# ecker-lab/TreeLearn

Measured on AMD Instinct MI355X. Metric: Mpoints/sec through sparse U-Net fwd (0.1 m voxel, 40x40 m tile), higher is better.
Workload: dtype bf16; 1 GPU; config2: single 40x40 m tile, voxel 0.1 m, 1890607 points/tile, 7-level 32-ch sparse U-Net fwd (30.1 M params, random init), 1 tile per GPU; points_per_tile=1890607, tiles_in_flight=4

## Files before the change

### treelearn_amd/csrc/tl_blk.hip

```cpp
#include "tl_common.h"

namespace {

constexpr int kBlock = 256;
constexpr int HASH = 2048;
constexpr uint32_t EMPTY = 0xFFFFFFFFu;
constexpr uint32_t KEYMASK = 0x01FFFFFFu;
constexpr int LIST = 128;

struct BlkGrid { int B, BX, BY, BZ, TX, TY; int64_t nblk; };

__device__ __forceinline__ void blk_decode(const BlkGrid& g, int64_t blk, int& b, int& bx, int& by, int& bz) {
  bz = (int)(blk % g.BZ); blk /= g.BZ;
  const int iy = (int)(blk & 3), ix = (int)((blk >> 2) & 3); blk >>= 4;
  const int ty = (int)(blk % g.TY); blk /= g.TY;
  const int tx = (int)(blk % g.TX);
  b = (int)(blk / g.TX);
  bx = tx * 4 + ix; by = ty * 4 + iy;
}

__device__ __forceinline__ uint32_t wg_exclusive_scan(uint32_t v, uint32_t* total) {
  __shared__ uint32_t wsum[kBlock / 64];
  const int lane = threadIdx.x & 63, wid = threadIdx.x >> 6;
  uint32_t inc = v;
  for (int off = 1; off < 64; off <<= 1) {
    const uint32_t t = (uint32_t)__shfl_up((int)inc, off);
    if (lane >= off) inc += t;
  }
  if (lane == 63) wsum[wid] = inc;
  __syncthreads();
  uint32_t base = 0, tot = 0;
  for (int w = 0; w < kBlock / 64; ++w) { if (w < wid) base += wsum[w]; tot += wsum[w]; }
  __syncthreads();
  *total = tot;
  return base + inc - v;
}

__global__ void __launch_bounds__(kBlock) k_blk_count(const uint64_t* __restrict__ bm, TlDims d, BlkGrid g, uint32_t* __restrict__ cnt,
                                                      uint32_t* __restrict__ part) {
  const int64_t blk = (int64_t)blockIdx.x * kBlock + threadIdx.x;
  uint32_t c = 0;
  if (blk < g.nblk) {
    int b, bx, by, bz;
    blk_decode(g, blk, b, bx, by, bz);
    const int sh = (bz & 7) * 8;
    for (int xi = 0; xi < 8; ++xi) {
      const int x = bx * 8 + xi;
      if (x >= d.X) break;
      for (int yi = 0; yi < 8; ++yi) {
        const int y = by * 8 + yi;
        if (y >= d.Y) break;
        const uint64_t w = bm[tl_col_word(d, b, x, y) + (bz >> 3)];
        c += __popc((uint32_t)(w >> sh) & 0xFFu);
      }
    }
    cnt[blk] = c;
  }
  uint32_t tot;
  wg_exclusive_scan(c, &tot);
  if (threadIdx.x == 0) part[blockIdx.x] = tot;
}

__global__ void __launch_bounds__(kBlock) k_blk_starts(const uint32_t* __restrict__ cnt, const uint32_t* __restrict__ part_excl, int64_t nblk,
                                                       uint32_t* __restrict__ bstart) {
  const int64_t blk = (int64_t)blockIdx.x * kBlock + threadIdx.x;
  const uint32_t c = blk < nblk ? cnt[blk] : 0;
  uint32_t tot;
  const uint32_t ex = wg_exclusive_scan(c, &tot);
  if (blk < nblk) bstart[blk] = part_excl[blockIdx.x] + ex;
}

__global__ void __launch_bounds__(1024) k_scan_u32(const uint32_t* __restrict__ in, int64_t n, uint32_t* __restrict__ out, uint32_t* __restrict__ total) {
  __shared__ uint32_t wsum[16];
  const int tid = threadIdx.x, lane = tid & 63, wid = tid >> 6;
  const int64_t per = (n + 1023) / 1024, lo = (int64_t)tid * per, hi = lo + per < n ? lo + per : n;
  uint32_t s = 0;
  for (int64_t i = lo; i < hi; ++i) s += in[i];
  uint32_t inc = s;
  for (int off = 1; off < 64; off <<= 1) {
    const uint32_t t = (uint32_t)__shfl_up((int)inc, off);
    if (lane >= off) inc += t;
  }
  if (lane == 63) wsum[wid] = inc;
  __syncthreads();
  uint32_t base = 0, tot = 0;
  for (int w = 0; w < 16; ++w) { if (w < wid) base += wsum[w]; tot += wsum[w]; }
  uint32_t run = base + inc - s;
  for (int64_t i = lo; i < hi; ++i) { const uint32_t v = in[i]; out[i] = run; run += v; }
  if (tid == 0 && total) *total = tot;
}

__global__ void __launch_bounds__(kBlock) k_blk_order(const uint64_t* __restrict__ bm, const uint32_t* __restrict__ pf, TlDims d, BlkGrid g,
                                                      const uint32_t* __restrict__ cnt, const uint32_t* __restrict__ bstart,
                                                      int32_t* __restrict__ o2n, int32_t* __restrict__ perm, int32_t* __restrict__ coords_new,
                                                      uint32_t* __restrict__ cs) {
  const int lane = threadIdx.x & 63;
  const int64_t blk = (int64_t)blockIdx.x * (kBlock / 64) + (threadIdx.x >> 6);
  if (blk >= g.nblk) return;
  if (cnt[blk] == 0) return;
  int b, bx, by, bz;
  blk_decode(g, blk, b, bx, by, bz);
  const int x = bx * 8 + (lane >> 3), y = by * 8 + (lane & 7);
  const bool valid = x < d.X && y < d.Y;
  const int sh = (bz & 7) * 8;
  uint64_t word = 0; int64_t w = 0;
  if (valid) { w = tl_col_word(d, b, x, y) + (bz >> 3); word = bm[w]; }
  uint32_t byte = (uint32_t)(word >> sh) & 0xFFu;
  const uint32_t pc = __popc(byte);
  uint32_t inc = pc;
  for (int off = 1; off < 64; off <<= 1) {
    const uint32_t t = (uint32_t)__shfl_up((int)inc, off);
    if (lane >= off) inc += t;
  }
  if (!pc) return;
  int newr = (int)(bstart[blk] + inc - pc);
  int old = (int)(pf[w] + __popcll(word & ((1ull << sh) - 1ull)));
  cs[(((int64_t)b * d.X + x) * d.Y + y) * g.BZ + bz] = (uint32_t)newr;
  while (byte) {
    const int zb = __ffs((int)byte) - 1;
    byte &= byte - 1;
    o2n[old] = newr; perm[newr] = old;
    reinterpret_cast<int4*>(coords_new)[newr] = make_int4(b, x, y, bz * 8 + zb);
    ++old; ++newr;
  }
}

struct BlkOut {
  const uint32_t* cs; int BZ;
  const int32_t* coords_new;
  int32_t* unit; int32_t* counter;
  int32_t* halo; uint32_t* lrb; int32_t* pmask; int32_t* nn_out;
  int64_t n; int64_t nchunks; int64_t cap_units; int halo_max;
};

__global__ void __launch_bounds__(kBlock) k_blk_units(const uint64_t* __restrict__ bm, TlDims d, BlkOut p) {
  __shared__ uint32_t s_tab[kBlock / 64][HASH + 64];
  __shared__ uint32_t s_list[kBlock / 64][LIST];
  __shared__ uint32_t s_lslot[kBlock / 64][LIST];
  const int lane = threadIdx.x & 63, wv = threadIdx.x >> 6;
  const int64_t chunk = (int64_t)blockIdx.x * (kBlock / 64) + wv;
  if (chunk >= p.nchunks) return;
  uint32_t* tab = s_tab[wv];
  uint32_t* list = s_list[wv];
  uint32_t* lslot = s_lslot[wv];
  const int64_t base = chunk * 64;
  const int cnt = (int)(p.n - base < 64 ? p.n - base : 64);
  const int64_t r = base + lane;
  const bool rvalid = lane < cnt;

  int nn[27];
#pragma unroll
  for (int k = 0; k < 27; ++k) nn[k] = -1;
  uint32_t pm = 0;
  {
    const int4 c = rvalid ? reinterpret_cast<const int4*>(p.coords_new)[r] : make_int4(0, 0, 0, 0);
    const int z = c.w;
    const bool hz0 = z > 0, hz2 = z + 1 < d.Z;
    const int bA = (hz0 ? z - 1 : z) >> 3, bB = (hz2 ? z + 1 : z) >> 3;
    const bool x0 = hz0 && ((z - 1) >> 6) != (z >> 6), x2 = hz2 && ((z + 1) >> 6) != (z >> 6);
    const int64_t wc0 = rvalid ? tl_col_word(d, c.x, c.y, c.z) : 0;
    const int64_t ci0 = rvalid ? (((int64_t)c.x * d.X + c.y) * d.Y + c.z) * p.BZ : 0;
    const bool xin[3] = {rvalid && c.y > 0, rvalid, rvalid && c.y + 1 < d.X}, yin[3] = {c.z > 0, true, c.z + 1 < d.Y};
    const int zw1 = rvalid ? (z >> 6) : 0, zw0 = (rvalid && x0) ? ((z - 1) >> 6) : zw1, zw2 = (rvalid && x2) ? ((z + 1) >> 6) : zw1;
    bool inb[9];
    uint64_t w1[9];
#pragma unroll
    for (int q = 0; q < 9; ++q) {
      const int dx = q / 3 - 1, dy = q % 3 - 1;
      inb[q] = xin[q / 3] && yin[q % 3];
      w1[q] = bm[wc0 + (inb[q] ? (dx * d.Y + dy) * d.Zw : 0) + zw1];
    }
    uint32_t by3[9];
#pragma unroll
    for (int q = 0; q < 9; ++q) {
      const uint32_t b1 = (uint32_t)(w1[q] >> (z & 56)) & 0xFFu;
      const uint32_t b0 = (uint32_t)(w1[q] >> ((hz0 ? z - 1 : z) & 56)) & 0xFFu, b2 = (uint32_t)(w1[q] >> ((hz2 ? z + 1 : z) & 56)) & 0xFFu;
      by3[q] = b0 | (b1 << 8) | (b2 << 16);
    }
    if (__any(x0 || x2)) {
#pragma unroll
      for (int q = 0; q < 9; ++q) {
        const int dx = q / 3 - 1, dy = q % 3 - 1;
        const int64_t wcq = wc0 + (inb[q] ? (dx * d.Y + dy) * d.Zw : 0);
        const uint64_t a0 = bm[wcq + zw0], a2 = bm[wcq + zw2];
        if (x0) by3[q] = (by3[q] & ~0xFFu) | ((uint32_t)(a0 >> ((z - 1) & 56)) & 0xFFu);
        if (x2) by3[q] = (by3[q] & ~0xFF0000u) | (((uint32_t)(a2 >> ((z + 1) & 56)) & 0xFFu) << 16);
      }
    }
    bool p0[9], p1[9], p2[9];
    uint32_t sA[9], sB[9];
#pragma unroll
    for (int q = 0; q < 9; ++q) {
      const int dx = q / 3 - 1, dy = q % 3 - 1;
      p0[q] = inb[q] && hz0 && ((by3[q] >> ((z - 1) & 7)) & 1u);
      p1[q] = inb[q] && ((by3[q] >> (8 + (z & 7))) & 1u);
      p2[q] = inb[q] && hz2 && ((by3[q] >> (16 + ((z + 1) & 7))) & 1u);
      const bool any = p0[q] || p1[q] || p2[q];
      const int64_t ciq = ci0 + (inb[q] ? (dx * d.Y + dy) * p.BZ : 0);
      sA[q] = p.cs[any ? ciq + bA : 0];
      sB[q] = p.cs[(any && bB != bA) ? ciq + bB : 0];
    }
    auto rowid = [](uint32_t byte, int zz, uint32_t start) __attribute__((always_inline)) {
      return (int)(start + __popc(byte & ((1u << (zz & 7)) - 1u)));
    };
#pragma unroll
    for (int q = 0; q < 9; ++q) {
      const uint32_t b_ = bB != bA ? sB[q] : sA[q];
      if (p0[q]) { nn[3 * q] = rowid(by3[q] & 0xFFu, z - 1, sA[q]); pm |= 1u << (3 * q); }
      if (p1[q]) { nn[3 * q + 1] = rowid((by3[q] >> 8) & 0xFFu, z, (z >> 3) == bA ? sA[q] : b_); pm |= 2u << (3 * q); }
      if (p2[q]) { nn[3 * q + 2] = rowid((by3[q] >> 16) & 0xFFu, z + 1, b_); pm |= 4u << (3 * q); }
    }
    if (rvalid) {
      p.pmask[r] = (int32_t)pm;
      if (p.nn_out) {
#pragma unroll
        for (int k = 0; k < 27; ++k) p.nn_out[(int64_t)k * p.n + r] = nn[k];
      }
    }
  }

  int nref = __popc(pm);
  for (int off = 32; off > 0; off >>= 1) nref += __shfl_xor(nref, off);
  const int TS = nref <= 360 ? 512 : (nref <= 720 ? 1024 : HASH);
  const int tshift = nref <= 360 ? 23 : (nref <= 720 ? 22 : 21);
  auto hs = [&](int v) __attribute__((always_inline)) { return ((uint32_t)v * 2654435761u) >> tshift; };

  int st_a[8], st_e[8];
  int sp = 1;
  st_a[0] = 0; st_e[0] = cnt;
  bool first = true;
  while (sp > 0) {
    --sp;
    const int a = st_a[sp], e = st_e[sp];
    const int lo = (int)base + a, hi = (int)base + e;
    for (int i = lane; i < TS; i += 64) tab[i] = EMPTY;
    __builtin_amdgcn_fence(__ATOMIC_ACQ_REL, "workgroup");
    const bool inr = lane >= a && lane < e;
    uint32_t outm = 0;
#pragma unroll
    for (int k = 0; k < 27; ++k) {
      const int v = nn[k];
      const bool out = inr && v >= 0 && (v < lo || v >= hi);
      outm |= out ? (1u << k) : 0u;
      tab[out ? hs(v) : (uint32_t)TS] = (uint32_t)v;
    }
    __builtin_amdgcn_fence(__ATOMIC_ACQ_REL, "workgroup");
    uint32_t lost = 0;
#pragma unroll
    for (int k = 0; k < 27; ++k) {
      const uint32_t cur = tab[hs(nn[k])];
      lost |= (((outm >> k) & 1u) && cur != (uint32_t)nn[k]) ? (1u << k) : 0u;
    }
    if (__any(lost != 0)) {
#pragma unroll
      for (int k = 0; k < 27; ++k) {
        bool todo = (lost >> k) & 1u;
        if (__any(todo)) {
          uint32_t s_ = hs(nn[k]);
          while (__any(todo)) {
            if (todo) {
              s_ = (s_ + 1) & (uint32_t)(TS - 1);
              if (tab[s_] == EMPTY) tab[s_] = (uint32_t)nn[k];
            }
            __builtin_amdgcn_fence(__ATOMIC_ACQ_REL, "workgroup");
            if (todo && tab[s_] == (uint32_t)nn[k]) todo = false;
            __builtin_amdgcn_fence(__ATOMIC_ACQ_REL, "workgroup");
          }
        }
      }
    }
    int H = 0;
    for (int i0 = 0; i0 < TS; i0 += 512) {
      uint32_t sv[8];
#pragma unroll
      for (int q = 0; q < 8; ++q) sv[q] = tab[i0 + q * 64 + lane];
#pragma unroll
      for (int q = 0; q < 8; ++q) {
        const unsigned long long m = __ballot(sv[q] != EMPTY);
        if (sv[q] != EMPTY) {
          const int at = H + __popcll(m & ((1ull << lane) - 1ull));
          if (at < LIST) { list[at] = sv[q]; lslot[at] = (uint32_t)(i0 + q * 64 + lane); }
        }
        H += __popcll(m);
      }
    }
    if (H > p.halo_max && e - a > 1) {
      const int mid = a + (e - a) / 2;
      st_a[sp] = mid; st_e[sp] = e; ++sp;
      st_a[sp] = a; st_e[sp] = mid; ++sp;
      continue;
    }
    int u;
    if (first) u = (int)chunk;
    else {
      int t = 0;
      if (lane == 0) t = atomicAdd(p.counter, 1);
      u = __shfl(t, 0);
    }
    first = false;
    if (u >= p.cap_units || H > LIST - 2) {
      if (lane == 0) atomicMax(p.counter + 1, 1);
      continue;
    }
    __builtin_amdgcn_fence(__ATOMIC_ACQ_REL, "workgroup");
    {
      const uint32_t k0 = lane < H ? list[lane] : EMPTY, s0 = lane < H ? lslot[lane] : (uint32_t)TS;
      int r0 = 0;
      const int H16 = (H + 15) & ~15;
      if (H <= 64) {
        for (int i = 0; i < H; ++i) r0 += (uint32_t)__builtin_amdgcn_readlane((int)k0, i) < k0 ? 1 : 0;
        if (lane < H) p.halo[(int64_t)lo * 32 + r0] = (int32_t)k0;
        tab[s0] = k0 | ((uint32_t)r0 << 25);
        if (lane >= H && lane < H16) p.halo[(int64_t)lo * 32 + lane] = -1;
      } else {
        const uint32_t k1 = lane + 64 < H ? list[lane + 64] : EMPTY, s1 = lane + 64 < H ? lslot[lane + 64] : (uint32_t)TS;
        int r1 = 0;
        for (int i = 0; i < 64; ++i) {
          const uint32_t b = (uint32_t)__builtin_amdgcn_readlane((int)k0, i);
          r0 += b < k0 ? 1 : 0; r1 += b < k1 ? 1 : 0;
        }
        for (int i = 64; i < H; ++i) {
          const uint32_t b = (uint32_t)__builtin_amdgcn_readlane((int)k1, i - 64);
          r0 += b < k0 ? 1 : 0; r1 += b < k1 ? 1 : 0;
        }
        p.halo[(int64_t)lo * 32 + r0] = (int32_t)k0;
        tab[s0] = k0 | ((uint32_t)r0 << 25);
        if (lane + 64 < H) p.halo[(int64_t)lo * 32 + r1] = (int32_t)k1;
        tab[s1] = k1 | ((uint32_t)r1 << 25);
        if (lane + 64 >= H && lane + 64 < H16) p.halo[(int64_t)lo * 32 + lane + 64] = -1;
      }
    }
    __builtin_amdgcn_fence(__ATOMIC_ACQ_REL, "workgroup");
    {
      uint32_t wds[9];
#pragma unroll
      for (int q = 0; q < 9; ++q) wds[q] = 0;
      uint32_t miss = 0;
      uint32_t cur[27];
#pragma unroll
      for (int k = 0; k < 27; ++k) cur[k] = tab[hs(nn[k])];
#pragma unroll
      for (int k = 0; k < 27; ++k) miss |= (((outm >> k) & 1u) && (cur[k] & KEYMASK) != (uint32_t)nn[k]) ? (1u << k) : 0u;
      if (__any(miss != 0)) {
#pragma unroll
        for (int k = 0; k < 27; ++k) {
          bool todo = (miss >> k) & 1u;
          if (__any(todo)) {
            uint32_t s_ = hs(nn[k]);
            while (__any(todo)) {
              if (todo) {
                s_ = (s_ + 1) & (uint32_t)(TS - 1);
                const uint32_t c_ = tab[s_];
                if ((c_ & KEYMASK) == (uint32_t)nn[k]) { cur[k] = c_; todo = false; }
              }
            }
          }
        }
      }
#pragma unroll
      for (int k = 0; k < 27; ++k) {
        const int v = nn[k];
        const bool out = (outm >> k) & 1u;
        const int pos = out ? 64 + (int)(cur[k] >> 25) : ((inr && v >= 0) ? v - lo : 191);
        const uint32_t val = (uint32_t)(pos * 4 + ((pos >> 2) & 3));
        wds[k / 3] |= val << ((k % 3) * 10);
      }
      if (inr) {
        uint32_t* dst = p.lrb + r * 9;
#pragma unroll
        for (int q = 0; q < 9; ++q) dst[q] = wds[q];
      }
    }
    if (lane == 0) reinterpret_cast<int4*>(p.unit)[u] = make_int4(lo, e - a, H, 0);
    __builtin_amdgcn_fence(__ATOMIC_ACQ_REL, "workgroup");
  }
}

__global__ void __launch_bounds__(kBlock) k_blk_tail_rank(int32_t* __restrict__ unit, const int32_t* __restrict__ counter, int nchunks, int64_t cap_units) {
  __shared__ int keys[kBlock];
  const int m = counter[0] - nchunks;
  if (m <= 1 || (int64_t)nchunks + 2 * (int64_t)m > cap_units) return;
  const int4* u = reinterpret_cast<const int4*>(unit) + nchunks;
  int4* tmp = reinterpret_cast<int4*>(unit) + (cap_units - m);
  for (int t0 = blockIdx.x * kBlock; t0 < m; t0 += gridDim.x * kBlock) {
    const int t = t0 + threadIdx.x;
    const int4 me = t < m ? u[t] : make_int4(0, 0, 0, 0);
    int rank = 0;
    for (int j0 = 0; j0 < m; j0 += kBlock) {
      keys[threadIdx.x] = j0 + (int)threadIdx.x < m ? u[j0 + threadIdx.x].x : 0x7FFFFFFF;
      __syncthreads();
      const int lim = m - j0 < kBlock ? m - j0 : kBlock;
      for (int j = 0; j < lim; ++j) rank += keys[j] < me.x ? 1 : 0;
      __syncthreads();
    }
    if (t < m) tmp[rank] = me;
  }
}
__global__ void __launch_bounds__(kBlock) k_blk_tail_copy(int32_t* __restrict__ unit, const int32_t* __restrict__ counter, int nchunks, int64_t cap_units) {
  const int m = counter[0] - nchunks;
  if (m <= 1 || (int64_t)nchunks + 2 * (int64_t)m > cap_units) return;
  const int4* tmp = reinterpret_cast<const int4*>(unit) + (cap_units - m);
  for (int t = blockIdx.x * kBlock + threadIdx.x; t < m; t += gridDim.x * kBlock) reinterpret_cast<int4*>(unit)[nchunks + t] = tmp[t];
}

__global__ void k_blk_init(int32_t* counter, int32_t nchunks) {
  if (threadIdx.x == 0) { counter[0] = nchunks; counter[1] = 0; }
}

}

extern "C" {

int64_t tl_blk_ws_words(const int32_t dims[4]) {
  if (!dims) return -1;
  const int64_t nblk = (int64_t)dims[0] * ((dims[1] + 31) / 32) * ((dims[2] + 31) / 32) * 16 * ((dims[3] + 7) / 8);
  const int64_t ncb = (int64_t)dims[0] * dims[1] * dims[2] * ((dims[3] + 7) / 8);
  return 2 * nblk + 2 * ((nblk + 255) / 256) + 8 + ncb;
}

int tl_blk_build(const uint64_t* bitmap, const uint32_t* prefix, const int32_t dims[4], int64_t n, const tl_blk* o, uint32_t* ws,
                 int phases, tl_stream_t stream) {
  if (!bitmap || !prefix || !dims || !o || !ws || n <= 0 || n >= (1 << 25) || !(phases & 3)) return TL_ERR_ARG;
  if (!o->o2n || !o->perm || !o->coords_new || !o->unit || !o->counter || !o->halo || !o->lrb || !o->pmask) return TL_ERR_ARG;
  if (o->halo_max < 26 || o->halo_max > TL_BLK_HALO_MAX || o->cap_units < (n + 63) / 64) return TL_ERR_ARG;
  if (((uintptr_t)o->unit) % 16 || ((uintptr_t)o->coords_new) % 16) return TL_ERR_ARG;
  const TlDims d = tl_dims(dims);
  BlkGrid g;
  g.B = d.B; g.BX = (d.X + 7) / 8; g.BY = (d.Y + 7) / 8; g.BZ = (d.Z + 7) / 8; g.TX = (g.BX + 3) / 4; g.TY = (g.BY + 3) / 4;
  g.nblk = (int64_t)g.B * g.TX * g.TY * 16 * g.BZ;
  hipStream_t s = tl_s(stream);
  uint32_t* cnt = ws;
  uint32_t* bstart = ws + g.nblk;
  const int64_t nparts = tl_cdiv(g.nblk, kBlock);
  uint32_t* part = ws + 2 * g.nblk;
  uint32_t* part_excl = part + nparts;
  uint32_t* cs = ws + 2 * g.nblk + 2 * nparts + 8;
  const int64_t nchunks = (n + 63) / 64;
  if (phases & 1) {
    k_blk_init<<<1, 64, 0, s>>>(o->counter, (int32_t)nchunks);
    k_blk_count<<<(unsigned)nparts, kBlock, 0, s>>>(bitmap, d, g, cnt, part);
    k_scan_u32<<<1, 1024, 0, s>>>(part, nparts, part_excl, part_excl + nparts);
    k_blk_starts<<<(unsigned)nparts, kBlock, 0, s>>>(cnt, part_excl, g.nblk, bstart);
    k_blk_order<<<(unsigned)tl_cdiv(g.nblk, kBlock / 64), kBlock, 0, s>>>(bitmap, prefix, d, g, cnt, bstart, o->o2n, o->perm, o->coords_new, cs);
  }
  if (!(phases & 2)) { TL_CHECK_LAUNCH(); return TL_OK; }
  BlkOut p;
  p.cs = cs; p.BZ = g.BZ; p.coords_new = o->coords_new; p.unit = o->unit; p.counter = o->counter; p.halo = o->halo; p.lrb = o->lrb; p.pmask = o->pmask; p.nn_out = o->nn;
  p.n = n; p.nchunks = nchunks; p.cap_units = o->cap_units; p.halo_max = o->halo_max;
  k_blk_units<<<(unsigned)tl_cdiv(nchunks, kBlock / 64), kBlock, 0, s>>>(bitmap, d, p);
  k_blk_tail_rank<<<32, kBlock, 0, s>>>(o->unit, o->counter, (int)nchunks, o->cap_units);
  k_blk_tail_copy<<<32, kBlock, 0, s>>>(o->unit, o->counter, (int)nchunks, o->cap_units);
  TL_CHECK_LAUNCH();
  return TL_OK;
}

}
```

Baseline: 268.5 Mpoints/s.

## Add bit-image fast path for halo construction in block units kernel

Adds a per-wavefront fast path for 64-row chunks whose voxels fit in a small x/y box with few z-bytes. It builds a column bit-image in LDS, derives halo bits with a dilation, and ranks halo rows by popcount prefix sums. This replaces the hash-table and recursive split halo construction. Chunks that do not fit fall back to the old hash path and are counted in a new counter slot. LDS is reorganised into one aliased per-wave buffer, and the extra register pressure may lower occupancy.

Result: no change. 269.6 Mpoints/s (median of 6 runs) (+0.4%).

```diff
diff --git a/treelearn_amd/csrc/tl_blk.hip b/treelearn_amd/csrc/tl_blk.hip
--- a/treelearn_amd/csrc/tl_blk.hip
+++ b/treelearn_amd/csrc/tl_blk.hip
@@ -7,6 +7,11 @@
 constexpr uint32_t EMPTY = 0xFFFFFFFFu;
 constexpr uint32_t KEYMASK = 0x01FFFFFFu;
 constexpr int LIST = 128;
+constexpr int WMEM = (HASH + 64 + 2 * LIST) / 2;
+constexpr int BI_COLS = 192, BI_NI = BI_COLS / 64, BI_BLKS = 16;
+constexpr int BI_C = 0, BI_H = BI_COLS, BI_S = 2 * BI_COLS, BI_HN = 3 * BI_COLS + 1, BI_PN = 4 * BI_COLS + 1, BI_TAB = 5 * BI_COLS + 1,
+              BI_LIST = BI_TAB + BI_BLKS, BI_END = BI_LIST + LIST / 2;
+static_assert(BI_END <= WMEM, "the bit-image path must fit the LDS the hash path uses");
 
 struct BlkGrid { int B, BX, BY, BZ, TX, TY; int64_t nblk; };
 
@@ -18,6 +23,8 @@
   b = (int)(blk / g.TX);
   bx = tx * 4 + ix; by = ty * 4 + iy;
 }
+
+__device__ __forceinline__ void lds_fence() { __builtin_amdgcn_fence(__ATOMIC_ACQ_REL, "workgroup", "local"); }
 
 __device__ __forceinline__ uint32_t wg_exclusive_scan(uint32_t v, uint32_t* total) {
   __shared__ uint32_t wsum[kBlock / 64];
@@ -134,15 +141,14 @@
 };
 
 __global__ void __launch_bounds__(kBlock) k_blk_units(const uint64_t* __restrict__ bm, TlDims d, BlkOut p) {
-  __shared__ uint32_t s_tab[kBlock / 64][HASH + 64];
-  __shared__ uint32_t s_list[kBlock / 64][LIST];
-  __shared__ uint32_t s_lslot[kBlock / 64][LIST];
+  __shared__ uint64_t s_mem[kBlock / 64][WMEM];
   const int lane = threadIdx.x & 63, wv = threadIdx.x >> 6;
   const int64_t chunk = (int64_t)blockIdx.x * (kBlock / 64) + wv;
   if (chunk >= p.nchunks) return;
-  uint32_t* tab = s_tab[wv];
-  uint32_t* list = s_list[wv];
-  uint32_t* lslot = s_lslot[wv];
+  uint64_t* mem = s_mem[wv];
+  uint32_t* tab = reinterpret_cast<uint32_t*>(mem);
+  uint32_t* list = tab + HASH + 64;
+  uint32_t* lslot = list + LIST;
   const int64_t base = chunk * 64;
   const int cnt = (int)(p.n - base < 64 ? p.n - base : 64);
   const int64_t r = base + lane;
@@ -152,11 +158,12 @@
 #pragma unroll
   for (int k = 0; k < 27; ++k) nn[k] = -1;
   uint32_t pm = 0;
+  const int4 c = rvalid ? reinterpret_cast<const int4*>(p.coords_new)[r] : make_int4(0, 0, 0, 0);
+  const int z = c.w;
+  const bool hz0 = z > 0, hz2 = z + 1 < d.Z;
+  const int bA = (hz0 ? z - 1 : z) >> 3, bB = (hz2 ? z + 1 : z) >> 3;
+  uint32_t ownbyte;
   {
-    const int4 c = rvalid ? reinterpret_cast<const int4*>(p.coords_new)[r] : make_int4(0, 0, 0, 0);
-    const int z = c.w;
-    const bool hz0 = z > 0, hz2 = z + 1 < d.Z;
-    const int bA = (hz0 ? z - 1 : z) >> 3, bB = (hz2 ? z + 1 : z) >> 3;
     const bool x0 = hz0 && ((z - 1) >> 6) != (z >> 6), x2 = hz2 && ((z + 1) >> 6) != (z >> 6);
     const int64_t wc0 = rvalid ? tl_col_word(d, c.x, c.y, c.z) : 0;
     const int64_t ci0 = rvalid ? (((int64_t)c.x * d.X + c.y) * d.Y + c.z) * p.BZ : 0;
@@ -177,6 +184,7 @@
       const uint32_t b0 = (uint32_t)(w1[q] >> ((hz0 ? z - 1 : z) & 56)) & 0xFFu, b2 = (uint32_t)(w1[q] >> ((hz2 ? z + 1 : z) & 56)) & 0xFFu;
       by3[q] = b0 | (b1 << 8) | (b2 << 16);
     }
+    ownbyte = (by3[4] >> 8) & 0xFFu;
     if (__any(x0 || x2)) {
 #pragma unroll
       for (int q = 0; q < 9; ++q) {
@@ -219,6 +227,201 @@
     }
   }
 
+  bool fast = false;
+  {
+    const int cntu = __builtin_amdgcn_readfirstlane(cnt);
+    const int x = c.y, y = c.z;
+    uint32_t rx = rvalid ? ((uint32_t)x | ((uint32_t)x << 16)) : 0x0000FFFFu;
+    uint32_t ry = rvalid ? ((uint32_t)y | ((uint32_t)y << 16)) : 0x0000FFFFu;
+    uint64_t zm = rvalid ? ((1ull << (bA & 63)) | (1ull << (bB & 63))) : 0ull;
+    uint32_t zl = (uint32_t)zm, zh = (uint32_t)(zm >> 32);
+    for (int off = 32; off > 0; off >>= 1) {
+      const uint32_t tx = (uint32_t)__shfl_xor((int)rx, off), ty = (uint32_t)__shfl_xor((int)ry, off);
+      rx = min(rx & 0xFFFFu, tx & 0xFFFFu) | (max(rx >> 16, tx >> 16) << 16);
+      ry = min(ry & 0xFFFFu, ty & 0xFFFFu) | (max(ry >> 16, ty >> 16) << 16);
+      zl |= (uint32_t)__shfl_xor((int)zl, off); zh |= (uint32_t)__shfl_xor((int)zh, off);
+    }
+    rx = (uint32_t)__builtin_amdgcn_readfirstlane((int)rx); ry = (uint32_t)__builtin_amdgcn_readfirstlane((int)ry);
+    const uint64_t zbm = (uint64_t)(uint32_t)__builtin_amdgcn_readfirstlane((int)zl) | ((uint64_t)(uint32_t)__builtin_amdgcn_readfirstlane((int)zh) << 32);
+    const int bfirst = __builtin_amdgcn_readfirstlane(c.x), blast = __builtin_amdgcn_readlane(c.x, cntu - 1);
+    const int xlo = (int)(rx & 0xFFFFu) - 1, xhi = (int)(rx >> 16) + 1, ylo = (int)(ry & 0xFFFFu) - 1, yhi = (int)(ry >> 16) + 1;
+    const int nx = xhi - xlo + 1, ny = yhi - ylo + 1, ncols = nx * ny;
+    const int bx0 = xlo >> 3, by0 = ylo >> 3, nby = (yhi >> 3) - by0 + 1, nB = ((xhi >> 3) - bx0 + 1) * nby;
+    const bool box = bfirst == blast && d.X < 65536 && d.Y < 65536 && p.BZ <= 64 && nx <= BI_COLS && ny <= BI_COLS && ncols <= BI_COLS &&
+                     nB <= BI_BLKS && __popcll(zbm) <= 8;
+    if (box) {
+      uint64_t* Cw = mem + BI_C; uint64_t* Hs = mem + BI_H; uint64_t* Sx = mem + BI_S; uint64_t* Hn = mem + BI_HN; uint64_t* Pn = mem + BI_PN;
+      uint2* btab = reinterpret_cast<uint2*>(mem + BI_TAB);
+      uint32_t* flist = reinterpret_cast<uint32_t*>(mem + BI_LIST);
+      const int lo = (int)base;
+      const uint32_t recip = (65536u + (uint32_t)ny - 1u) / (uint32_t)ny;
+      int cxr[BI_NI], cyr[BI_NI]; bool cing[BI_NI]; uint64_t Oc[BI_NI];
+      {
+        int64_t wc[BI_NI];
+#pragma unroll
+        for (int i = 0; i < BI_NI; ++i) {
+          const int n = i * 64 + lane < ncols ? i * 64 + lane : 0;
+          cxr[i] = (int)(((uint32_t)n * recip) >> 16); cyr[i] = n - cxr[i] * ny;
+          const int gx = xlo + cxr[i], gy = ylo + cyr[i];
+          cing[i] = gx >= 0 && gx < d.X && gy >= 0 && gy < d.Y;
+          wc[i] = cing[i] ? tl_col_word(d, bfirst, gx, gy) : 0;
+          Oc[i] = 0;
+        }
+        uint64_t rest = zbm;
+        int s_ = 0;
+        while (rest) {
+          const int w = (__ffsll((unsigned long long)rest) - 1) >> 3;
+          uint64_t word[BI_NI];
+#pragma unroll
+          for (int i = 0; i < BI_NI; ++i) word[i] = i * 64 < ncols ? bm[wc[i] + w] : 0ull;
+          uint32_t bits = (uint32_t)(rest >> (8 * w)) & 0xFFu;
+          rest &= ~(0xFFull << (8 * w));
+          while (bits) {
+            const int f = __ffs((int)bits) - 1, len = __ffs((int)~(bits >> f)) - 1;
+            const uint64_t m = len >= 8 ? ~0ull : ((1ull << (8 * len)) - 1ull);
+#pragma unroll
+            for (int i = 0; i < BI_NI; ++i) Oc[i] |= ((word[i] >> (8 * f)) & m) << (8 * s_);
+            s_ += len;
+            bits &= ~(((1u << len) - 1u) << f);
+          }
+        }
+      }
+      {
+        const int t = lane < nB ? lane : 0;
+        const int bxr = t / nby, byr = t - bxr * nby, bx = bx0 + bxr, by = by0 + byr;
+        const int key = lane < nB ? (((bx >> 2) * 16384 + (by >> 2)) * 16 + (bx & 3) * 4 + (by & 3)) : 0x7FFFFFFF;
+        const int xs = max(bx * 8, xlo), xe = min(bx * 8 + 7, xhi), ys = max(by * 8, ylo), ye = min(by * 8 + 7, yhi);
+        const int wy = ye - ys + 1, area = lane < nB ? (xe - xs + 1) * wy : 0;
+        int cb = 0;
+        for (int i = 0; i < nB; ++i) cb += __builtin_amdgcn_readlane(key, i) < key ? __builtin_amdgcn_readlane(area, i) : 0;
+        if (lane < nB) btab[lane] = make_uint2((uint32_t)cb | ((uint32_t)area << 16), (uint32_t)(xs - xlo) | ((uint32_t)(ys - ylo) << 8) | ((uint32_t)wy << 16));
+#pragma unroll
+        for (int i = 0; i < BI_NI; ++i)
+          if (i * 64 < ncols) Cw[i * 64 + lane] = 0;
+      }
+      lds_fence();
+      auto slot_of = [&](int zb) __attribute__((always_inline)) { return __popcll(zbm & ((1ull << (zb & 63)) - 1ull)); };
+      const int n0 = rvalid ? (x - xlo) * ny + (y - ylo) : ny + 1;
+      const int sA = slot_of(bA);
+      if (rvalid) {
+        const uint32_t below = (1u << (z & 7)) - 1u;
+        if (lane == 0 || !(ownbyte & below)) {
+          uint32_t m = ownbyte & ~below;
+          const int L = min(__popc(m), cnt - lane);
+          while (__popc(m) > L) m &= ~(0x80000000u >> __clz(m));
+          reinterpret_cast<uint8_t*>(Cw)[n0 * 8 + ((z >> 3) == bA ? sA : sA + 1)] = (uint8_t)m;
+        }
+      }
+      lds_fence();
+      int mycol[BI_NI]; uint32_t myfa[BI_NI];
+      int hsum = 0;
+#pragma unroll
+      for (int i = 0; i < BI_NI; ++i) {
+        mycol[i] = 0; myfa[i] = 0;
+        if (i * 64 < ncols) {
+          const bool act = i * 64 + lane < ncols, ing = cing[i];
+          const int n = act ? i * 64 + lane : 0;
+          const int xr = cxr[i], yr = cyr[i], gx = xlo + xr, gy = ylo + yr;
+          const uint64_t O = Oc[i];
+          uint64_t D = 0, own = 0;
+#pragma unroll
+          for (int q = 0; q < 9; ++q) {
+            const uint64_t w = Cw[min(max(n + (q / 3 - 1) * ny + (q % 3 - 1), 0), ncols - 1)];
+            D |= w;
+            if (q == 4) own = w;
+          }
+          D |= (D << 1) | (D >> 1);
+          const uint64_t h = (act && ing) ? (D & O & ~own) : 0ull;
+          {
+            const uint2 e = btab[((gx >> 3) - bx0) * nby + ((gy >> 3) - by0)];
+            myfa[i] = e.x;
+            mycol[i] = min((int)(e.x & 0xFFFFu) + (xr - (int)(e.y & 0xFFu)) * (int)((e.y >> 16) & 0xFFu) + (yr - (int)((e.y >> 8) & 0xFFu)), BI_COLS - 1);
+          }
+          if (act) { Hs[mycol[i]] = h; Hn[n] = h; }
+          hsum += __popcll(h);
+        }
+      }
+      for (int off = 32; off > 0; off >>= 1) hsum += __shfl_xor(hsum, off);
+      const int H = __builtin_amdgcn_readfirstlane(hsum);
+      if (H <= p.halo_max && H <= LIST - 2) {
+        lds_fence();
+        {
+          uint64_t v[BI_NI], tot = 0;
+#pragma unroll
+          for (int i = 0; i < BI_NI; ++i) {
+            uint64_t h = lane * BI_NI + i < ncols ? Hs[lane * BI_NI + i] : 0ull;
+            h = h - ((h >> 1) & 0x5555555555555555ull);
+            h = (h & 0x3333333333333333ull) + ((h >> 2) & 0x3333333333333333ull);
+            v[i] = (h + (h >> 4)) & 0x0F0F0F0F0F0F0F0Full;
+            tot += v[i];
+          }
+          uint64_t inc = tot;
+          for (int off = 1; off < 64; off <<= 1) {
+            const uint32_t tl_ = (uint32_t)__shfl_up((int)(uint32_t)inc, off), th_ = (uint32_t)__shfl_up((int)(uint32_t)(inc >> 32), off);
+            if (lane >= off) inc += (uint64_t)tl_ | ((uint64_t)th_ << 32);
+          }
+          uint64_t run = inc - tot;
+#pragma unroll
+          for (int i = 0; i < BI_NI; ++i) { Sx[lane * BI_NI + i] = run; run += v[i]; }
+          if (lane == 63) Sx[BI_COLS] = inc;
+        }
+        lds_fence();
+#pragma unroll
+        for (int i = 0; i < BI_NI; ++i) {
+          if (i * 64 < ncols) {
+            const int cb = min((int)(myfa[i] & 0xFFFFu), BI_COLS), ce = min(cb + (int)(myfa[i] >> 16), BI_COLS);
+            const uint64_t sb = Sx[cb], se = Sx[ce], sc = Sx[mycol[i]];
+            uint64_t tb = sb, ts = se - sb;
+            tb += tb << 8; tb += tb << 16; tb += tb << 32;
+            ts += ts << 8; ts += ts << 16; ts += ts << 32;
+            const uint32_t bt = (uint32_t)(tb >> 56) * 0x01010101u;
+            if (i * 64 + lane < ncols) Pn[i * 64 + lane] = ((uint64_t)bt | ((uint64_t)bt << 32)) + (ts << 8) + (sc - sb);
+          }
+        }
+        lds_fence();
+        {
+          uint32_t wds[9];
+          int shl[3]; uint32_t bel[3];
+#pragma unroll
+          for (int t = 0; t < 3; ++t) {
+            shl[t] = ((z + t - 1) >> 3) != bA && (t == 1 || (t == 2 && hz2)) ? 8 : 0;
+            bel[t] = ((1u << ((z + t - 1) & 7)) - 1u) << shl[t];
+          }
+#pragma unroll
+          for (int q = 0; q < 9; ++q) {
+            const int nq = n0 + (q / 3 - 1) * ny + (q % 3 - 1);
+            const uint32_t hw = (uint32_t)(Hn[nq] >> (8 * sA)), pw = (uint32_t)(Pn[nq] >> (8 * sA));
+            uint32_t wd = 0;
+#pragma unroll
+            for (int t = 0; t < 3; ++t) {
+              const int v = nn[3 * q + t];
+              const int rank = (int)((pw >> shl[t]) & 0xFFu) + __popc(hw & bel[t]);
+              const uint32_t u = (uint32_t)(v - lo);
+              const bool inside = u < (uint32_t)cnt, out = v >= 0 && !inside;
+              flist[out ? (rank & (LIST - 1)) : LIST - 1] = (uint32_t)v;
+              const int pos = inside ? (int)u : (out ? 64 + rank : 191);
+              wd |= (uint32_t)(pos * 4 + ((pos >> 2) & 3)) << (t * 10);
+            }
+            wds[q] = wd;
+          }
+          if (rvalid) {
+            uint32_t* dst = p.lrb + r * 9;
+#pragma unroll
+            for (int q = 0; q < 9; ++q) dst[q] = wds[q];
+          }
+        }
+        lds_fence();
+        const int H16 = (H + 15) & ~15;
+        if (lane < H16) p.halo[(int64_t)lo * 32 + lane] = lane < H ? (int32_t)flist[lane] : -1;
+        if (lane + 64 < H16) p.halo[(int64_t)lo * 32 + lane + 64] = lane + 64 < H ? (int32_t)flist[lane + 64] : -1;
+        if (lane == 0) reinterpret_cast<int4*>(p.unit)[chunk] = make_int4(lo, cnt, H, 0);
+        fast = true;
+      }
+      lds_fence();
+    }
+  }
+  if (!fast && lane == 0) atomicAdd(p.counter + 2, 1);
+
   int nref = __popc(pm);
   for (int off = 32; off > 0; off >>= 1) nref += __shfl_xor(nref, off);
   const int TS = nref <= 360 ? 512 : (nref <= 720 ? 1024 : HASH);
@@ -226,7 +429,7 @@
   auto hs = [&](int v) __attribute__((always_inline)) { return ((uint32_t)v * 2654435761u) >> tshift; };
 
   int st_a[8], st_e[8];
-  int sp = 1;
+  int sp = fast ? 0 : 1;
   st_a[0] = 0; st_e[0] = cnt;
   bool first = true;
   while (sp > 0) {
@@ -404,7 +607,7 @@
 }
 
 __global__ void k_blk_init(int32_t* counter, int32_t nchunks) {
-  if (threadIdx.x == 0) { counter[0] = nchunks; counter[1] = 0; }
+  if (threadIdx.x == 0) { counter[0] = nchunks; counter[1] = 0; counter[2] = 0; }
 }
 
 }
```
